# LSimon95/megatts2

Hardware: AMD Instinct MI355X
Metric: mel-frames/sec (whole node) (higher is better)
Workload: dtype f32; 1 GPU; C3: B=32/GPU x 1 GPU, Np=70, Tp=431, Tm=431; stages vqpe+mrte+adm+plm+decoder+vocoder; forced durations; weights=synthetic (name-seeded), parallelism=dp1 (utterance shards, one RCCL all-gather of mels per step)

## Files before the change

### include/megatts2_hip.h

```cpp
#ifndef MEGATTS2_HIP_H
#define MEGATTS2_HIP_H

#include <stddef.h>
#include <stdint.h>

#ifdef __cplusplus
extern "C" {
#endif

typedef struct mt2_model mt2_model;

typedef struct mt2_config {
    int32_t mel_bins, mrte_hidden, mrte_kernel, mrte_stride, mrte_n_layer, mrte_n_stack, mrte_n_block;
    int32_t content_ff_dim, content_n_heads, content_n_layers, phone_vocab;
    int32_t vq_mel_bins, vq_stride, vq_hidden, vq_kernel, vq_n_layers, vq_n_stacks, vq_n_blocks, vq_bins, vq_dim;
    int32_t dec_kernel, dec_hidden, dec_n_stack, dec_n_block;
    int32_t plm_layers, plm_heads, plm_vq_dim, plm_tc_dim, plm_bins;
    int32_t adm_layers, adm_heads, adm_emb_dim, adm_tc_dim, adm_tc_emb_dim;
    int32_t hg_in_dim, hg_init_channels, hg_n_up, hg_up_rates[8], hg_up_kernels[8];
    int32_t hg_n_res, hg_res_kernels[4], hg_res_dilations[4][3];
    float hg_slope;
    int32_t max_positions;
    int32_t hg_inference_padding;
    int32_t hg_reflect_pad;
// ... 230 lines not shown
enum { MT2_ATTN_NONE = 0, MT2_ATTN_GENERIC = 1, MT2_ATTN_REG = 2, MT2_ATTN_DS = 3, MT2_ATTN_LDS = 4, MT2_ATTN_X6 = 5, MT2_ATTN_X3H = 6 };
typedef struct mt2_attn_desc {
    int32_t struct_bytes;
    const float* Q; int32_t ldq;
    const float* K; int32_t ldk;
    const float* V; int32_t ldv;
    float* O; int32_t ldo;
    const int32_t* q_start; const int32_t* q_len; const int32_t* kv_start; const int32_t* kv_len; const int32_t* o_start;
    int32_t u_qstride, u_qlen, u_kvstride, u_kvlen, u_ostride;
    int32_t B, H, D, max_qlen, max_kvlen; float scale;
    int32_t lds_min_qlen, x6_min_qlen, lds_waves, ds_short, x3h, o_planes;
    int32_t* range_flag;
    int32_t* kernel_out;
} mt2_attn_desc;
int mt2_op_attention_desc(void* stream, const mt2_attn_desc* d);
int mt2_attention_route(const mt2_attn_desc* d, int32_t* err, int32_t* kernel, int32_t* tmpl, int32_t* launch, long long* lds);
int mt2_gemm_trace_begin(mt2_model* m);
int mt2_gemm_trace_end(mt2_model* m, int cap, const char** names, int64_t* launches, double* flops, double* ms);
int mt2_gemm_trace_shapes(mt2_model* m, char* buf, int cap, int top);
int mt2_gemm_config_count(void);
const char* mt2_gemm_config_name(int idx);
int mt2_gemm_route(int M, int N, int K, int taps, int dil, int groups, int pro_act, int operands, int misaligned, int force_cfg,
                   int x3h, int* err, int* cfg, int* variant, long long* lds, int* planes);
int mt2_op_gemm_x3h_ln(void* stream, const float* X, int ldx, int Rx, int a_mul, int shift0, const float* W, const void* W3,
                       const void* Wh, const float* wh_inv, const float* bias, const float* R, int ldr, float* C, int ldc, int M, int N,
                       int K, int epi_act, int force_cfg, float* stat_out, int32_t* stat_nt, int32_t* stat_w, const float* ln_stat,
                       int ln_nt, int ln_w, const float* ln_s, float ln_eps);
int mt2_bench_gemm(void* stream, int M, int N, int K, int taps, int dil, int flags, int force_cfg, int iters,
                   int w_copies, float* avg_ms, char* cfg_name, int cfg_name_cap, double* sustained_ghz);

#ifdef __cplusplus
}
#endif
#endif
```

### megatts2_amd/csrc/capi.inc

```

#include <climits>

namespace mt2 {
extern thread_local std::string g_last_error;
void finalize_model(mt2_model& m);
}

using namespace mt2;

#define MT2_API_BEGIN try {
#define MT2_API_END                                 \
    ::CallScope::verdict_of_open_call();            \
    return 0;                                       \
    }                                               \
    catch (const std::exception& e) {               \
        g_last_error = e.what();                    \
        return -1;                                  \
    }                                               \
    catch (...) {                                   \
        g_last_error = "unknown error";             \
        return -1;                                  \
    }

enum Need { NEED_G = 1, NEED_ADM = 2, NEED_PLM = 4, NEED_VOC = 8 };
// ... 248 lines not shown
    if (n == "ar_groups") return &m->ar_groups;
    if (n == "adm_groups") return &m->adm_groups;
    if (n == "plm_groups") return &m->plm_groups;
    if (n == "force_gemm_config") return &m->opts.force_cfg;
    if (n == "t_ks4") return &m->opts.t_ks4;
    if (n == "t_ks2") return &m->opts.t_ks2;
    if (n == "t32") return &m->opts.t32;
    if (n == "t32x32") return &m->opts.t32x32;
    if (n == "t_x6_256") return &m->opts.t_x6_256;
    if (n == "t_x6_128") return &m->opts.t_x6_128;
    if (n == "t_x3h_128") return &m->opts.t_x3h_128;
    if (n == "x3h") return &m->opts.x3h;
    if (n == "x6_ks") return &m->opts.x6_ks;
    if (n == "voc_streams") return &m->opts.voc_streams;
    if (n == "ldr_prio") return &m->opts.ldr_prio;
    if (n == "skinny_rows") return &m->opts.skinny_rows;
    if (n == "skinny_nw") return &m->opts.skinny_nw;
    if (n == "skinny_pairs") return &m->opts.skinny_pairs;
    if (n == "attn_lds_min") return &m->opts.attn_lds_min;
    if (n == "attn_x6_min") return &m->opts.attn_x6_min;
    if (n == "ln_pairs_adm") return &m->opts.ln_pairs_adm;
    if (n == "ln_pairs_maxm") return &m->opts.ln_pairs_maxm;
    if (n == "a_planes") return &m->opts.a_planes;
    return nullptr;
}
static bool* option_flag(mt2_model* m, const std::string& n) {
    if (n == "splitk") return &m->opts.splitk;
    if (n == "stage_markers") return &m->opts.markers;
    if (n == "win_conv") return &m->opts.win_conv;
    if (n == "x6_conv") return &m->opts.x6_conv;
    if (n == "x6_gemm") return &m->opts.x6_gemm;
    if (n == "skinny_tm") return &m->opts.skinny_tm;
    if (n == "ldr64") return &m->opts.ldr64;
    return nullptr;
}
int mt2_set_option(mt2_model* m, const char* name, int value) {
    MT2_API_BEGIN
    MT2_REQUIRE(m != nullptr && name != nullptr, "null argument");
    std::lock_guard<std::mutex> lk(m->call_mutex);
    const std::string n(name);
    if (n == "ar_groups") MT2_REQUIRE(value >= 1 && value <= 8, "ar_groups must be in 1..8");
    if (int* p = option_slot(m, n)) *p = value;
    else if (bool* q = option_flag(m, n)) *q = value != 0;
    else throw Error("unknown option " + n);
    MT2_API_END
}
// ... 790 lines not shown
    p.X = (const float*)ptr(0, 512); p.ldx = Cin; p.Rx = M + taps * dil; p.a_mul = 1; p.taps = taps; p.dil = dil; p.Cin = Cin;
    p.W = (const float*)ptr(1, 0); p.ldw = K; p.C = (float*)ptr(2, 1024); p.ldc = N; p.M = M; p.N = N; p.K = K; p.groups = groups;
    p.strideX = (long long)p.Rx * Cin; p.strideW = (long long)N * K; p.strideC = (long long)M * N; p.strideB = N; p.strideR = (long long)M * N;
    p.pro_act = pro_act; p.out_scale = 1.0f;
    if (operands & 1) p.W3 = ptr(3, 1);
    if (operands & 2) { p.Wh = ptr(4, 2); p.wh_inv = (const float*)ptr(5, 0); }
    if (operands & 4) { p.Wtm = (const float*)ptr(6, 4); p.tm_kb = K / 64; }
    if (operands & 8) p.stat_out = (float*)ptr(7, 8);
    if (operands & 16) { p.ln_stat = (const float*)ptr(8, 16); p.ln_g = p.ln_b = (const float*)ptr(9, 0); p.ln_w = 64; p.ln_nt = K / 64; }
    if (operands & 32) { p.R = (const float*)ptr(10, 32); p.ldr = N; }
    if (operands & 64) p.rowbase = (const int*)ptr(11, 64);
    p.a_planes = (operands & 128) ? 1 : 0;
    p.c_planes = (operands & 256) ? 1 : 0;
    EngineOpts o;
    o.force_cfg = force_cfg;
    o.x3h = x3h;
    const GemmRoute r = gemm_route(p, o);
    if (err) *err = (int)r.err;
    if (cfg) *cfg = r.cfg;
    if (variant) *variant = r.variant;
    if (lds) *lds = (long long)r.lds;
    if (planes) *planes = (gemm_takes_planes(p, o) ? 1 : 0) | (gemm_writes_planes(p, o) ? 2 : 0);
    return 0;
}

int mt2_op_gemm(void* stream, const float* X, int ldx, int Rx, const int32_t* rowbase, int a_mul, int shift0,
                int taps, int dil, int Cin, const float* W, int ldw, const float* bias, const float* R, int ldr,
                const int32_t* valid, float* C, int ldc, int M, int N, int pro_act, float pro_slope, int epi_act,
                float out_scale, int force_cfg) {
    MT2_API_BEGIN
    GemmP p{};
    p.X = X; p.ldx = ldx; p.Rx = Rx; p.rowbase = rowbase; p.a_mul = a_mul ? a_mul : 1; p.shift0 = shift0;
    p.taps = taps; p.dil = dil; p.Cin = Cin; p.W = W; p.ldw = ldw; p.bias = bias; p.R = R; p.ldr = ldr;
    p.valid = valid; p.C = C; p.ldc = ldc; p.M = M; p.N = N; p.K = taps * Cin; p.groups = 1;
    p.pro_act = pro_act; p.pro_slope = pro_slope; p.epi_act = epi_act; p.out_scale = out_scale;
    EngineOpts o;
    o.force_cfg = force_cfg;
    MT2_HIP(launch_gemm(p, (hipStream_t)stream, &o));
    MT2_API_END
}

int mt2_op_gemm_x6(void* stream, const float* X, int ldx, int Rx, int shift0, int taps, int dil, int Cin, const float* W,
                   const void* W3, const float* bias, const float* R, int ldr, const int32_t* valid, float* C, int ldc,
                   int M, int N, int pro_act, float pro_slope, int epi_act, int force_cfg) {
    MT2_API_BEGIN
    GemmP p{};
// ... 522 lines not shown
```

### megatts2_amd/csrc/gemm_x3h.hip

```cpp
#include "gemm_common.h"

#include <atomic>

#ifndef MT2_X3H_ABLATE
#define MT2_X3H_ABLATE 0
#endif
#define MT2_ABL_NOINGEST (MT2_X3H_ABLATE == 2 || MT2_X3H_ABLATE == 5 || MT2_X3H_ABLATE == 6 || MT2_X3H_ABLATE == 7)
#define MT2_ABL_NOSPLIT (MT2_X3H_ABLATE == 3 || MT2_X3H_ABLATE == 5 || MT2_X3H_ABLATE == 6)
#define MT2_ABL_NOBARRIER (MT2_X3H_ABLATE == 6 || MT2_X3H_ABLATE == 7)
#ifdef MT2_X3H_NO_BUFFER_LOADS
#define MT2_BUFFER_LOADS false
#else
#define MT2_BUFFER_LOADS true
#endif

namespace mt2 {

typedef _Float16 f16x8 __attribute__((ext_vector_type(8)));
typedef _Float16 f16x2 __attribute__((ext_vector_type(2)));
typedef float f32x2 __attribute__((ext_vector_type(2)));
typedef unsigned u32x4 __attribute__((ext_vector_type(4)));

constexpr float kX3hLoScale = 2048.0f, kX3hLoInv = 1.0f / 2048.0f, kX3hMaxIn = 65504.0f;

// ... 999 lines not shown
                    __builtin_amdgcn_s_barrier();
                    asm volatile("" ::: "memory");
                }
                fetch_a(b, sa, swza);
                fetch_b(b, sb);
                __builtin_amdgcn_sched_barrier(0);
            }
        }
        stn = stn + 1 == NST ? 0 : stn + 1;
        if (++qn == QS) { qn = 0; ++tapn; }
    };
    for (int c = 0; c + 1 < nk; ++c) chunk(std::false_type{});
    chunk(std::true_type{});
#pragma unroll
    for (int i = 0; i < TM; ++i)
#pragma unroll
        for (int j = 0; j < TN; ++j)
#pragma unroll
            for (int e = 0; e < 16; ++e) acc[i][j][e] = __builtin_fmaf(acl[i][j][e], kX3hLoInv, acc[i][j][e]) * inv_s[j];
    if (epilogue_t4_ok(p)) epilogue_t4<TM, TN>(p, acc, 0, m0 + wm * WTM, wn * WTN, lane);
    else epilogue<TM, TN>(p, acc, 0, m0 + wm * WTM, wn * WTN, lane);
}


#define MT2_X3H_LDR(IDX_, BM_, BN_, WM_, WN_, NL_, NST_)                                                                    \
    { IDX_, BM_, BN_, (WM_* WN_ + NL_) * 64, (size_t)NST_ * ((size_t)BM_ * BK * 4 + (size_t)(2 * BN_ / 16) * 1024),         \
      "x3hldr" #BM_ "x" #BN_ "_" #WM_ "x" #WN_ "+" #NL_ "_s" #NST_ "xc",                                                    \
      { gemm_x3h_ldr_kernel<BM_, BN_, WM_, WN_, NL_, NST_, ACT_NONE>, gemm_x3h_ldr_kernel<BM_, BN_, WM_, WN_, NL_, NST_, ACT_RELU>, \
        gemm_x3h_ldr_kernel<BM_, BN_, WM_, WN_, NL_, NST_, ACT_LRELU>, gemm_x3h_ldr_kernel<BM_, BN_, WM_, WN_, NL_, NST_, PRO_APL>, \
        gemm_x3h_ldr_kernel<BM_, BN_, WM_, WN_, NL_, NST_, PRO_LNX> }, PIPE_X3H, 0, 0, (BN_) / (WN_) }
#define MT2_X3H_KS(IDX_, BM_, BN_, WM_, WN_, KS_, NL_, NST_)                                                                \
    { IDX_, BM_, BN_, (WM_* WN_ * KS_ + NL_) * 64, (size_t)KS_ * NST_ * ((size_t)BM_ * BK * 4 + (size_t)(2 * BN_ / 16) * 1024), \
      "x3hks" #BM_ "x" #BN_ "_" #WM_ "x" #WN_ "_k" #KS_ "+" #NL_ "_s" #NST_,                                                \
      { gemm_x3h_ks_kernel<BM_, BN_, WM_, WN_, KS_, NL_, NST_, ACT_NONE>, gemm_x3h_ks_kernel<BM_, BN_, WM_, WN_, KS_, NL_, NST_, ACT_RELU>, \
        gemm_x3h_ks_kernel<BM_, BN_, WM_, WN_, KS_, NL_, NST_, ACT_LRELU>, gemm_x3h_ks_kernel<BM_, BN_, WM_, WN_, KS_, NL_, NST_, PRO_APL>, \
        gemm_x3h_ks_kernel<BM_, BN_, WM_, WN_, KS_, NL_, NST_, PRO_LNX> }, PIPE_X3H, 0, KS_, 32 }
#define MT2_X3H_WIN(IDX_, QS_, BM_, BN_, WM_, WN_, NST_, NL_)                                                               \
    { IDX_, BM_, BN_, (WM_* WN_ + NL_) * 64, (size_t)NST_ * (((2 * BN_ / 16 + NL_ - 1) / NL_) * NL_ * 1024),                  \
      "x3hwin" #BM_ "x" #BN_ "_" #WM_ "x" #WN_ "+" #NL_ "_s" #NST_,                                                          \
      { conv_win_x3h_kernel<QS_, BM_, BN_, WM_, WN_, NST_, ACT_NONE, NL_>, conv_win_x3h_kernel<QS_, BM_, BN_, WM_, WN_, NST_, ACT_RELU, NL_>, \
        conv_win_x3h_kernel<QS_, BM_, BN_, WM_, WN_, NST_, ACT_LRELU, NL_> }, PIPE_X3H, QS_ }

static const TileCfg kX3hRows[] = {
    MT2_X3H_KS(CFG_X3HKS32x64_K4, 32, 64, 1, 2, 4, 8, 2),
    MT2_X3H_KS(CFG_X3HKS64x64_K2, 64, 64, 2, 2, 2, 8, 3),
    MT2_X3H_KS(CFG_X3HKS32x32_K8, 32, 32, 1, 1, 8, 8, 2),
// ... 9 lines not shown
```

### megatts2_amd/csrc/model_stages.hip

```cpp
#include "mt2_model.h"
#include "x3h_planes.h"
#include "gemm_tiles.h"

#include <algorithm>
#include <cmath>
#include <cstring>
#include <numeric>

namespace mt2 {



static RowSet make_rows(const int* lens, int B, int G) {
    RowSet rs;
    rs.B = B; rs.G = G;
    rs.len.assign(lens, lens + B);
    rs.off.resize(B);
    int r = G;
    for (int b = 0; b < B; ++b) {
        MT2_REQUIRE(lens[b] >= 0, "negative utterance length");
        rs.off[b] = r;
        r += lens[b] + G;
        rs.maxlen = std::max(rs.maxlen, lens[b]);
    }
// ... 149 lines not shown
    }
    const bool planes = linear_takes_planes(c, h_scratch, K, M, w.W, w.bias, N, K, y, ldy, epi_act);
    LnP q{};
    q.x = x + (long long)shift0 * ldx; q.ldx = ldx * p.a_mul; q.gamma = w.g; q.beta = w.b; q.out = h_scratch; q.ldo = K;
    q.M = M; q.C = K; q.eps = 1e-5f; q.act = ACT_NONE; q.out_planes = planes ? 1 : 0; q.x3h_flag = c.m.opts.x3h_flag;
    MT2_HIP(launch_layernorm(q, c.s));
    linear(c, h_scratch, K, M, w.W, w.bias, N, K, y, ldy, nullptr, 0, nullptr, epi_act, planes, c_planes);
}
static LnOps ln1_qkv(const EncLayerW& w, int d, int n0 = 0) {
    return ln_ops(w.ln1g, w.ln1b, w.wqkv, w.bqkv, w.wqkv_l, w.sqkv, w.cqkv, n0, d);
}
static LnOps ln2_ff0(const EncLayerW& w, int d) {
    return ln_ops(w.ln2g, w.ln2b, w.ff0w, w.ff0b, w.ff0_l, w.sff0, w.cff0, 0, d);
}

static void conv_same(const Ctx& c, const float* x, int ldx, int R, const ConvW& w, float* y, int ldy,
                      const int* valid, int pro_act = ACT_NONE, float slope = 0.f, int epi_act = ACT_NONE,
                      const float* Rsd = nullptr, int ldr = 0, int dil = 1) {
    GemmP p{};
    p.X = x; p.ldx = ldx; p.Rx = R; p.taps = w.k; p.dil = dil; p.shift0 = -((w.k - 1) / 2) * dil; p.Cin = w.cin;
    p.W = w.w; p.bias = w.b; p.R = Rsd; p.ldr = ldr; p.valid = valid; p.C = y; p.ldc = ldy; p.M = R; p.N = w.cout;
    p.pro_act = pro_act; p.pro_slope = slope; p.epi_act = epi_act;
    gemm(c, p);
}

static void layernorm(const Ctx& c, const float* x, int ldx, const float* g, const float* b, int M, int C,
                      float* out, int ldo, const int* valid = nullptr, int valid_rows = 0,
                      const float* R1 = nullptr, int ldr1 = 0, int r1_rows = 0, int rows_per_group = 0,
                      int act = ACT_NONE, bool out_planes = false) {
    LnP p{};
    p.x = x; p.ldx = ldx; p.gamma = g; p.beta = b; p.rows_per_group = rows_per_group;
    p.R1 = R1; p.ldr1 = ldr1; p.r1_rows = r1_rows; p.valid = valid; p.valid_rows = valid_rows;
    p.out = out; p.ldo = ldo; p.M = M; p.C = C; p.eps = 1e-5f; p.act = act;
    p.out_planes = out_planes ? 1 : 0; p.x3h_flag = c.m.opts.x3h_flag;
    MT2_HIP(launch_layernorm(p, c.s));
}

static float* run_stack(const Ctx& c, const StackW& w, const float* x_in, bool shared_in, int R,
                        const int* valid) {
    const int C = w.C, G = w.groups;
    const size_t per = (size_t)R * C;
    float* T = c.ws.get<float>(per * G);
    float* Y = c.ws.get<float>(per * G);
    float* XA = c.ws.get<float>(per * G);
    float* XB = c.ws.get<float>(per * G);
    const float* cur = x_in;
// ... 991 lines not shown
        const int nside = m.opts.voc_streams > 1 ? 2 : 0;
        ensure_aux(m, nside);
        if (reflect) {
            int g0 = 0;
            for (int j = 0; j < 3; ++j) g0 = std::max(g0, (m.hg_res[i * 3 + j].k - 1) / 2 * m.hg_res[i * 3 + j].dil[0]);
            halo(c, up, ch, g0);
        }
        if (nside) {
            MT2_HIP(hipEventRecord(m.ev_fork, c.s));
            m.aux_forked = true;
            for (int j = 0; j < nside; ++j) MT2_HIP(hipStreamWaitEvent(m.aux_streams[j], m.ev_fork, 0));
        }
        for (int j = 0; j < 3; ++j) {
            const ResW& r = m.hg_res[i * 3 + j];
            const Ctx cj{m, (nside && j > 0) ? m.aux_streams[j - 1] : c.s, c.ws};
            float* t1 = c.ws.get<float>(per);
            float* ha = c.ws.get<float>(per);
            float* hb = c.ws.get<float>(per);
            rb[j] = c.ws.get<float>(per);
            const float* h = up;
            for (int n = 0; n < 3; ++n) {
                float* out = n == 2 ? rb[j] : (n == 0 ? ha : hb);
                if (n > 0) halo(cj, const_cast<float*>(h), ch, (r.k - 1) / 2 * r.dil[n]);
                conv_same(cj, h, ch, (int)R, r.c1[n], t1, ch, valid, ACT_LRELU, slope, ACT_LRELU, nullptr, 0, r.dil[n]);
                halo(cj, t1, ch, (r.k - 1) / 2);
                conv_same(cj, t1, ch, (int)R, r.c2[n], out, ch, valid, ACT_NONE, slope, ACT_NONE, h, ch, 1);
                h = out;
            }
        }
        for (int j = 0; j < nside; ++j) {
            MT2_HIP(hipEventRecord(m.ev_join[j], m.aux_streams[j]));
            MT2_HIP(hipStreamWaitEvent(c.s, m.ev_join[j], 0));
        }
        if (!reflect && i + 1 == cfg.hg_n_up && m.hg_post.cout == 1 && (ch & 3) == 0 && ch <= 128 && m.hg_post.k <= 15) {
            float* wav = c.ws.get<float>((size_t)R);
            const hipError_t e = launch_conv_post(rb[0], rb[1], rb[2], 1.0f / 3.0f, R, ch, m.hg_post.k, m.hg_post.w,
                                                  m.hg_post.b, 0.01f, valid, wav, c.s);
            if (e == hipSuccess) return wav;
            if (e != hipErrorNotSupported) MT2_HIP(e);
        }
        x = c.ws.get<float>(per);
        MT2_HIP(launch_avg3(rb[0], rb[1], rb[2], 1.0f / 3.0f, x, (long long)per, c.s));
    }
    float* wav = c.ws.get<float>((size_t)R);
    halo(c, x, ch, (m.hg_post.k - 1) / 2);
    conv_same(c, x, ch, (int)R, m.hg_post, wav, 1, valid, ACT_LRELU, 0.01f, ACT_TANH);
// ... 617 lines not shown
```

### megatts2_amd/csrc/mt2_kernels.h

```cpp
#pragma once
#include <hip/hip_runtime.h>
#include <stdint.h>

#include <atomic>
#include <vector>

namespace mt2 {

inline hipError_t dyn_lds_once(std::atomic<unsigned long long>& done, const void* fn, size_t bytes) {
    int dev = 0;
    hipError_t e = hipGetDevice(&dev);
    if (e != hipSuccess) return e;
    const unsigned long long bit = 1ull << (dev & 63);
    if (done.load(std::memory_order_acquire) & bit) return hipSuccess;
    e = hipFuncSetAttribute(fn, hipFuncAttributeMaxDynamicSharedMemorySize, (int)bytes);
    if (e != hipSuccess) return e;
    done.fetch_or(bit, std::memory_order_release);
    return hipSuccess;
}

constexpr int kInvalidRow = -(1 << 30);

enum Act : int { ACT_NONE = 0, ACT_RELU = 1, ACT_LRELU = 2, ACT_TANH = 3,
                 ACT_LOGCLAMP = 4 };
// ... 20 lines not shown
    const float* Wtm = nullptr;
    int tm_n0 = 0, tm_k0 = 0;
    int tm_kb = 0;
    const float* bias; long long strideB;
    const float* R; long long strideR; int ldr;
    const int* valid;
    float* C; long long strideC; int ldc;
    int M, N, K, groups;
    int pro_act; float pro_slope; int epi_act; float out_scale;
    const float* ln_g; const float* ln_b; float ln_eps;
    float* stat_out = nullptr; int stat_nt = 0, stat_w = 0;
    const float* ln_stat = nullptr; int ln_nt = 0, ln_w = 0;
};
struct TraceRec { int cfg; double flops; hipEvent_t e0, e1; int M, N, K, groups; };
struct EngineOpts {
    int force_cfg = -1;
    int t_ks4 = 256, t_ks2 = 640, t32 = 64, t32x32 = 160;
    bool splitk = true;
    int voc_streams = 3;
    bool win_conv = true;
    bool x6_conv = true;
    bool x6_gemm = true;
    int x3h = 15;
    int* x3h_flag = nullptr;
    int t_x3h_128 = 72;
    int t_x6_256 = 160, t_x6_128 = 72;
    int x6_ks = 4;
    int a_planes = 3;
    bool ldr64 = false;
    int ldr_prio = 3;
    int skinny_rows = 64;
    int attn_lds_min = 640;
    int attn_x6_min = 192;
    bool skinny_tm = true;
    int skinny_pairs = 1;
    int skinny_nw = 16;
    bool markers = false;
    bool trace_on = false;
    std::vector<TraceRec> trace;
    const char* last_cfg = "";
    int last_stat_nt = 0, last_stat_w = 0;
    int ln_pairs = 0;
    int ln_pairs_adm = 2;
    int ln_pairs_maxk = 1024;
    int ln_pairs_maxm = 1280;
};
struct GemmRoute { hipError_t err; int cfg; int variant; size_t lds; int stat_nt, stat_w; };
GemmRoute gemm_route(const GemmP& p, const EngineOpts& o);
hipError_t launch_gemm(const GemmP& p, hipStream_t s, EngineOpts* o = nullptr);
bool gemm_takes_planes(const GemmP& p, const EngineOpts& o);
bool gemm_writes_planes(const GemmP& p, const EngineOpts& o);
bool gemm_skinny_eligible(const GemmP& p, int max_rows);
hipError_t launch_gemm_skinny(const GemmP& p, hipStream_t s);
bool gemm_skinny_tm_eligible(const GemmP& p, int max_rows);
hipError_t launch_gemm_skinny_tm(const GemmP& p, hipStream_t s);
hipError_t launch_tile_major(const float* W, int N, int K, float* out, hipStream_t s);
int gemm_num_configs();
const char* gemm_config_name(int idx);
int gemm_trace_collect(EngineOpts& o, int cap, const char** names, int64_t* launches, double* flops, double* ms);
int gemm_trace_shapes(EngineOpts& o, char* buf, int cap, int top);

struct LnP {
    const float* x; int ldx;
    const float* gamma; const float* beta; int rows_per_group;
    const float* R1; int ldr1; int r1_rows; const float* R2; int ldr2;
    const int* valid; int valid_rows;
    float* out; int ldo;
    int M, C; float eps; int act;
    int out_planes = 0;
    int* x3h_flag = nullptr;
};
hipError_t launch_layernorm(const LnP& p, hipStream_t s);
// ... 196 lines not shown
```

### megatts2_amd/runtime.py

```python
from __future__ import annotations

import ctypes as C
import math
import os
from typing import Dict, Optional, Sequence

import numpy as np

from . import config as cfgmod
from . import sampling as sampmod

_LIB = None
MAX_POSITIONS = 8192

MT2_RUN_PLM, MT2_RUN_VOCODER, MT2_SKIP_ADM, MT2_PROMPT_VQPE = 1, 2, 4, 8
ACT_NONE, ACT_RELU, ACT_LRELU, ACT_TANH = 0, 1, 2, 3
ACT_LOGCLAMP = 4
MT2_RESAMPLE_NORMALIZE = 1
TRIM_FRAME, TRIM_HOP = 2048, 512
F0_FRAME, F0_WINDOW, F0_MAX_LAG = 1024, 768, 256
DTW_MAX_LEN, DTW_DIR_COLS = 4096, 16


class NativeError(RuntimeError):
# ... 908 lines not shown
    inv = torch.empty(w.shape[0], dtype=torch.float32)
    _check(lib.mt2_x3h_split(C.c_void_p(w.data_ptr()), C.c_longlong(w.shape[0]), C.c_longlong(w.shape[1]),
                             C.c_void_p(planes.data_ptr()), C.c_void_p(inv.data_ptr())))
    return planes, inv


def op_conv_x3h(X, W, bias=None, R=None, valid=None, shift0=0, taps=1, dil=1, Cin=None, pro_act=ACT_NONE, pro_slope=0.0,
                epi_act=ACT_NONE, force_cfg=-1, want_flag=False):
    import torch
    lib = load_library()
    Cin = Cin or X.shape[1]
    N, M = W.shape[0], X.shape[0]
    W3 = split_bf16x3(W).to(X.device)
    ph, inv = split_f16x2_rows(W)
    ph, inv = ph.to(X.device), inv.to(X.device)
    out = torch.empty(M, N, device=X.device, dtype=torch.float32)
    flag = torch.zeros(4, device=X.device, dtype=torch.int32)
    _check(lib.mt2_op_gemm_x3h(_stream(), _ptr(X), X.shape[1], M, shift0, taps, dil, Cin, _ptr(W), _ptr(W3), _ptr(ph), _ptr(inv),
                               _ptr(bias), _ptr(R), R.shape[1] if R is not None else 0, _ptr(valid), _ptr(out), N, M, N, pro_act,
                               C.c_float(pro_slope), epi_act, force_cfg, _ptr(flag)))
    return (out, int(flag[0].item())) if want_flag else out


def op_gemm_x6_ln(X, W, bias=None, R=None, M=None, a_mul=1, shift0=0, epi_act=ACT_NONE, force_cfg=-1, want_stats=False,
                  ln=None, eps=1e-5, x3h=False):
    import torch
    lib = load_library()
    K, N = X.shape[1], W.shape[0]
    M = M or X.shape[0]
    dev = X.device
    out = torch.empty(M, N, device=dev, dtype=torch.float32)
    stat = torch.zeros(M, 32, 2, device=dev, dtype=torch.float32) if want_stats else None
    nt, pw = C.c_int32(0), C.c_int32(0)
    ln_stat, ln_nt, ln_w, ln_s = None, 0, 0, None
    if ln is not None:
        gamma, beta, pairs, ln_w = ln
        Wd = W.double().cpu()
        Wl = (W.cpu() * gamma.cpu()[None, :]).to(torch.float32)
        ln_s = Wl.double().sum(1).to(torch.float32).to(dev)
        bias = (Wd @ beta.double().cpu() + (bias.double().cpu() if bias is not None else 0.0)).to(torch.float32).to(dev)
        W = Wl.to(dev)
        ln_stat = pairs.contiguous()
        ln_nt = pairs.shape[1]
    W = W.contiguous()
    W3 = split_bf16x3(W).to(dev)
    if x3h:
# ... 348 lines not shown
```

Measured before the change: 78320 mel-frames/s.

## Fuse HiFiGAN resblock conv pairs into one x3h kernel keeping intermediate in LDS

Adds a conv_pair kernel that runs a resblock's two consecutive convolutions (leaky-relu conv with dilation, then conv plus residual) in one launch. The intermediate activation stays in LDS as f16 hi/lo planes, and dedicated loader waves stream both weight sets. This removes one launch, the global write and read of the intermediate, and the halo pass. The cost is recomputing overlapping rows at tile edges (output tile BM-(taps-1)). The path is on by default for 32- and 64-channel resblocks (pair_fuse=3) and falls back to the old path when a case is unsupported.

```diff
diff --git a/include/megatts2_hip.h b/include/megatts2_hip.h
--- a/include/megatts2_hip.h
+++ b/include/megatts2_hip.h
@@ -276,6 +276,11 @@
 const char* mt2_gemm_config_name(int idx);
 int mt2_gemm_route(int M, int N, int K, int taps, int dil, int groups, int pro_act, int operands, int misaligned, int force_cfg,
                    int x3h, int* err, int* cfg, int* variant, long long* lds, int* planes);
+int mt2_conv_pair_route(int R, int C, int taps, int dil, int flags, int pair_fuse, int x3h, int* err, long long* lds, int* grid,
+                        int* block, int* bm, int* bmo);
+int mt2_op_conv_pair(void* stream, const float* X, int ldx, int R, int C, int taps, int dil, float slope, const void* Wh1,
+                     const float* inv1, const float* bias1, const void* Wh2, const float* inv2, const float* bias2,
+                     const int32_t* valid, float* Y, int ldy, int pair_fuse, int32_t* range_flag);
 int mt2_op_gemm_x3h_ln(void* stream, const float* X, int ldx, int Rx, int a_mul, int shift0, const float* W, const void* W3,
                        const void* Wh, const float* wh_inv, const float* bias, const float* R, int ldr, float* C, int ldc, int M, int N,
                        int K, int epi_act, int force_cfg, float* stat_out, int32_t* stat_nt, int32_t* stat_w, const float* ln_stat,
diff --git a/megatts2_amd/csrc/capi.inc b/megatts2_amd/csrc/capi.inc
--- a/megatts2_amd/csrc/capi.inc
+++ b/megatts2_amd/csrc/capi.inc
@@ -294,6 +294,7 @@
     if (n == "ln_pairs_adm") return &m->opts.ln_pairs_adm;
     if (n == "ln_pairs_maxm") return &m->opts.ln_pairs_maxm;
     if (n == "a_planes") return &m->opts.a_planes;
+    if (n == "pair_fuse") return &m->opts.pair_fuse;
     return nullptr;
 }
 static bool* option_flag(mt2_model* m, const std::string& n) {
@@ -1130,6 +1131,45 @@
     if (lds) *lds = (long long)r.lds;
     if (planes) *planes = (gemm_takes_planes(p, o) ? 1 : 0) | (gemm_writes_planes(p, o) ? 2 : 0);
     return 0;
+}
+
+int mt2_conv_pair_route(int R, int C, int taps, int dil, int flags, int pair_fuse, int x3h, int* err, long long* lds, int* grid,
+                        int* block, int* bm, int* bmo) {
+    alignas(128) static char dummy[8 * 128];
+    PairP p{};
+    p.X = (const float*)dummy; p.ldx = C; p.R = R; p.C = C; p.taps = taps; p.dil = dil; p.slope = 0.1f;
+    if (!(flags & 2)) { p.Wh1 = dummy + 128; p.inv1 = (const float*)(dummy + 256); p.Wh2 = dummy + 384; p.inv2 = (const float*)(dummy + 512); }
+    p.bias1 = (const float*)(dummy + 640); p.bias2 = (const float*)(dummy + 768);
+    p.wh_ldb = 4ll * (((long long)taps * C + 31) / 32 * 32);
+    p.Y = (float*)(dummy + 896 + ((flags & 8) ? 4 : 0)); p.ldy = C;
+    p.reflect = (flags & 1) ? 1 : 0;
+    if ((flags & 4) && R > 0) p.ldx = (int)((((1ll << 31) / 4 + R - 1) / R + 3) & ~3ll);
+    EngineOpts o;
+    o.pair_fuse = pair_fuse;
+    o.x3h = x3h;
+    const PairRoute r = conv_pair_route(p, o);
+    if (err) *err = (int)r.err;
+    if (lds) *lds = (long long)r.lds;
+    if (grid) *grid = (int)r.grid;
+    if (block) *block = (int)r.block;
+    if (bm) *bm = r.bm;
+    if (bmo) *bmo = r.bmo;
+    return 0;
+}
+int mt2_op_conv_pair(void* stream, const float* X, int ldx, int R, int C, int taps, int dil, float slope, const void* Wh1,
+                     const float* inv1, const float* bias1, const void* Wh2, const float* inv2, const float* bias2,
+                     const int32_t* valid, float* Y, int ldy, int pair_fuse, int32_t* range_flag) {
+    MT2_API_BEGIN
+    PairP p{};
+    p.X = X; p.ldx = ldx; p.R = R; p.C = C; p.taps = taps; p.dil = dil; p.slope = slope;
+    p.Wh1 = Wh1; p.inv1 = inv1; p.bias1 = bias1; p.Wh2 = Wh2; p.inv2 = inv2; p.bias2 = bias2;
+    p.wh_ldb = 4ll * (((long long)taps * C + 31) / 32 * 32);
+    p.valid = valid; p.Y = Y; p.ldy = ldy;
+    EngineOpts o;
+    o.pair_fuse = pair_fuse;
+    o.x3h_flag = range_flag;
+    MT2_HIP(launch_conv_pair(p, (hipStream_t)stream, &o));
+    MT2_API_END
 }
 
 int mt2_op_gemm(void* stream, const float* X, int ldx, int Rx, const int32_t* rowbase, int a_mul, int shift0,
diff --git a/megatts2_amd/csrc/gemm_x3h.hip b/megatts2_amd/csrc/gemm_x3h.hip
--- a/megatts2_amd/csrc/gemm_x3h.hip
+++ b/megatts2_amd/csrc/gemm_x3h.hip
@@ -1045,6 +1045,375 @@
     else epilogue<TM, TN>(p, acc, 0, m0 + wm * WTM, wn * WTN, lane);
 }
 
+template <int PRO, int QS, int NT, int MAXT>
+__device__ __forceinline__ void pair_rows_to_planes(float* win, int tid, int WRp, int nrows, float slope, float& amax) {
+    const unsigned lds_w = (unsigned)(unsigned long long)(__attribute__((address_space(3))) float*)win;
+    const int ntask = QS * nrows * 4;
+    f32x4 in[MAXT][2];
+    int rbk_[MAXT];
+    __builtin_amdgcn_s_barrier();
+    asm volatile("" ::: "memory");
+#pragma unroll
+    for (int u = 0; u < MAXT; ++u) {
+        const int t = tid + u * NT;
+        const int tt = t < ntask ? t : 0;
+        const int rr = tt >> 2, j = tt & 3;
+        const int q = rr / nrows, row = rr - q * nrows;
+        const int rbk = q * WRp + row;
+        rbk_[u] = rbk;
+        const int swz = (row >> 1) & 7;
+        const unsigned base = lds_w + (unsigned)rbk * 128;
+        in[u][0] = lds_read_b128(base + (unsigned)(((2 * j) ^ swz) * 16));
+        in[u][1] = lds_read_b128(base + (unsigned)(((2 * j + 1) ^ swz) * 16));
+    }
+    asm volatile("s_waitcnt lgkmcnt(0)" ::: "memory");
+#pragma unroll
+    for (int u = 0; u < MAXT; ++u) asm volatile("" : "+v"(in[u][0]), "+v"(in[u][1]));
+    __builtin_amdgcn_s_barrier();
+    asm volatile("" ::: "memory");
+#pragma unroll
+    for (int u = 0; u < MAXT; ++u) {
+        const int t = tid + u * NT;
+        if (t < ntask) {
+            const int j = t & 3, rbk = rbk_[u];
+            const int swz = ((rbk % WRp) >> 1) & 7;
+            u32x4 ph, pl;
+            split2_f16<PRO>(in[u][0], in[u][1], slope, ph, pl, amax);
+            char* dst = reinterpret_cast<char*>(win) + (size_t)rbk * 128;
+            *reinterpret_cast<u32x4*>(dst + ((j ^ swz) * 16)) = ph;
+            *reinterpret_cast<u32x4*>(dst + (((4 + j) ^ swz) * 16)) = pl;
+        }
+    }
+    asm volatile("s_waitcnt lgkmcnt(0)" ::: "memory");
+}
+
+template <int QS, int BM, int BN, int WGM, int WGN, int NST, int NL>
+__global__ __launch_bounds__((WGM * WGN + NL) * 64) void conv_pair_x3h_kernel(PairP p) {
+    constexpr int NW = WGM * WGN;
+    constexpr int WTM = BM / WGM, WTN = BN / WGN;
+    constexpr int TM = WTM / 32, TN = WTN / 32;
+    constexpr int BPIECES = BN / 8;
+    constexpr int NI = NL;
+    constexpr int B_IT = (BPIECES + NI - 1) / NI;
+    constexpr int STAGE_B = B_IT * NI * 1024;
+    constexpr int NT = (NW + NL) * 64;
+    constexpr int MAXT1 = (QS * (BM + 64) * 4 + NT - 1) / NT;
+    constexpr int MAXT2 = (QS * BM * 4 + NT - 1) / NT;
+    static_assert(NL > 0 && WTM % 32 == 0 && WTN % 32 == 0 && NST >= 3 && (NST - 2) * B_IT < 64 && BN == 32 * QS, "config");
+
+    extern __shared__ __attribute__((aligned(16))) float smem[];
+    const int tid = threadIdx.x, lane = tid & 63;
+    const int wave_all = __builtin_amdgcn_readfirstlane(tid >> 6);
+    const bool loader = wave_all >= NW;
+    const int wave = loader ? wave_all - NW : wave_all;
+    const int wm = wave / WGN, wn = wave % WGN;
+    const int taps = p.taps;
+    const int WR = BM + (taps - 1) * p.dil, WRp = (WR + 7) & ~7;
+    const int BMo = BM - (taps - 1);
+    char* ring = reinterpret_cast<char*>(smem);
+    float* win = smem + NST * STAGE_B / 4;
+
+    const int ntm = (p.R + BMo - 1) / BMo;
+    const int bid = blockIdx.x;
+    const int xcd = bid & 7, qq = ntm >> 3, rr = ntm & 7;
+    const int tile = (xcd < rr ? xcd * (qq + 1) : rr * (qq + 1) + (xcd - rr) * qq) + (bid >> 3);
+    const int o0 = tile * BMo;
+    const int t0 = o0 - (taps - 1) / 2;
+
+    const float* __restrict__ X = p.X;
+    const long long zoff_x = (const float*)g_zero16 - X;
+    const int ldx = p.ldx, Rx = p.R;
+    {
+        const int lrow = lane >> 3;
+        const int ppq = WRp >> 3, pieces = QS * ppq;
+        const int row_first = t0 - (taps - 1) / 2 * p.dil;
+        for (int pc = wave_all; pc < pieces; pc += NW + NL) {
+            const int q = pc / ppq, r8 = pc - q * ppq;
+            const int row = r8 * 8 + lrow;
+            const int grow = row_first + row;
+            const int slot = (lane & 7) ^ ((row >> 1) & 7);
+            const bool ok = (row < WR) & ((unsigned)grow < (unsigned)Rx);
+            const long long off = ok ? (long long)grow * ldx + q * 32 + slot * 4 : zoff_x;
+            __builtin_amdgcn_global_load_lds((const __attribute__((address_space(1))) void*)(X + off),
+                                             (__attribute__((address_space(3))) void*)(win + (q * WRp + r8 * 8) * 32), 16, 0, 0);
+        }
+    }
+    const int nk = taps * QS;
+    constexpr unsigned kOut = 0x80000000u;
+    unsigned vob[B_IT];
+#pragma unroll
+    for (int j = 0; j < B_IT; ++j) {
+        const int pc = j * NI + wave;
+        const int n = pc * 8 + (lane >> 3);
+        const int sl = (lane & 7) ^ ((n >> 1) & 7);
+        vob[j] = (pc < BPIECES && n < BN) ? (unsigned)(n * (int)p.wh_ldb + sl * 16) : kOut;
+    }
+    auto issue = [&](const __amdgpu_buffer_rsrc_t& rs, int c, int st) __attribute__((always_inline)) {
+        char* Bs = ring + st * STAGE_B + wave * 1024;
+#pragma unroll
+        for (int j = 0; j < B_IT; ++j)
+            __builtin_amdgcn_raw_ptr_buffer_load_lds(rs, (__attribute__((address_space(3))) void*)(Bs + j * NI * 1024), 16, (int)vob[j], c * 128, 0, 0);
+    };
+    auto loader_loop = [&](const __amdgpu_buffer_rsrc_t& rs) __attribute__((always_inline)) {
+        for (int c = 0; c < nk; ++c) {
+            if (c == 0) { if (NST - 2 < nk) wait_vmcnt<(NST - 2) * B_IT>(); else wait_vmcnt<0>(); }
+            else if (c + NST - 3 < nk) wait_vmcnt<(NST - 3) * B_IT>();
+            else wait_vmcnt<0>();
+            __builtin_amdgcn_s_barrier();
+            if (c >= 1 && c + NST - 2 < nk) issue(rs, c + NST - 2, (c + NST - 2) % NST);
+        }
+    };
+    if (loader) {
+        const __amdgpu_buffer_rsrc_t rs1 = __builtin_amdgcn_make_buffer_rsrc(const_cast<char*>(reinterpret_cast<const char*>(p.Wh1)), 0, (int)kOut, 0x00020000);
+        const __amdgpu_buffer_rsrc_t rs2 = __builtin_amdgcn_make_buffer_rsrc(const_cast<char*>(reinterpret_cast<const char*>(p.Wh2)), 0, (int)kOut, 0x00020000);
+        loader_priority(p.ldr_prio);
+#pragma unroll
+        for (int st = 0; st < NST - 1; ++st)
+            if (st < nk) issue(rs1, st, st);
+        if (nk >= NST - 1) wait_vmcnt<(NST - 1) * B_IT>();
+        else wait_vmcnt<0>();
+        float amax = 0.0f;
+        pair_rows_to_planes<ACT_LRELU, QS, NT, MAXT1>(win, tid, WRp, WRp, p.slope, amax);
+        if (p.x3h_flag != nullptr && __builtin_amdgcn_ballot_w64(amax >= kX3hMaxIn) != 0ull && lane == 0) atomicOr(p.x3h_flag, 1);
+        loader_loop(rs1);
+        __builtin_amdgcn_s_barrier();
+        asm volatile("" ::: "memory");
+#pragma unroll
+        for (int st = 0; st < NST - 1; ++st)
+            if (st < nk) issue(rs2, st, st);
+        amax = 0.0f;
+        pair_rows_to_planes<ACT_NONE, QS, NT, MAXT2>(win, tid, WRp, BM, p.slope, amax);
+        if (p.x3h_flag != nullptr && __builtin_amdgcn_ballot_w64(amax >= kX3hMaxIn) != 0ull && lane == 0) atomicOr(p.x3h_flag, 1);
+        loader_loop(rs2);
+        return;
+    }
+    unsigned vmask[TM];
+    {
+        int vv[TM];
+#pragma unroll
+        for (int i = 0; i < TM; ++i) {
+            const int g = t0 + wm * WTM + i * 32 + (lane & 31);
+            const bool ok = (unsigned)g < (unsigned)Rx;
+            vv[i] = ok ? (p.valid ? p.valid[g] : 1) : 0;
+        }
+        wait_vmcnt<0>();
+#pragma unroll
+        for (int i = 0; i < TM; ++i) vmask[i] = (unsigned)__builtin_amdgcn_ballot_w64(vv[i] != 0);
+    }
+    float amax = 0.0f;
+    pair_rows_to_planes<ACT_LRELU, QS, NT, MAXT1>(win, tid, WRp, WRp, p.slope, amax);
+    if (p.x3h_flag != nullptr && __builtin_amdgcn_ballot_w64(amax >= kX3hMaxIn) != 0ull && lane == 0) atomicOr(p.x3h_flag, 1);
+
+    f32x16 acc[TM][TN], acl[TM][TN];
+    const int half = lane >> 5;
+    const unsigned lds_ring = (unsigned)(unsigned long long)(__attribute__((address_space(3))) char*)ring;
+    const unsigned lds_win = (unsigned)(unsigned long long)(__attribute__((address_space(3))) float*)win;
+    const int nrow = wn * WTN + (lane & 31);
+    const unsigned b_lane = lds_ring + nrow * 128;
+    const int swzb = (nrow >> 1) & 7;
+    unsigned koffb[2][2];
+#pragma unroll
+    for (int b = 0; b < 2; ++b) {
+        koffb[b][0] = (unsigned)(((b * 2 + half) ^ swzb) * 16);
+        koffb[b][1] = (unsigned)(((4 + b * 2 + half) ^ swzb) * 16);
+    }
+    const int arow0 = wm * WTM + (lane & 31);
+    constexpr int N1 = 2 * TM + 2 * TN;
+    static_assert(N1 <= 15, "lgkmcnt is four bits wide");
+    u32x4 ra[2][TM][2];
+    u32x4 rb[2][2][TN];
+    auto fetch_a = [&](int b, unsigned sa, int swza) __attribute__((always_inline)) {
+        const unsigned vh = sa + (unsigned)(((b * 2 + half) ^ swza) * 16), vl = sa + (unsigned)(((4 + b * 2 + half) ^ swza) * 16);
+        static_for(std::make_integer_sequence<int, TM>{}, [&](auto ic) {
+            constexpr int i = decltype(ic)::value;
+            ra[b][i][0] = __builtin_bit_cast(u32x4, lds_read_b128_imm<i * 32 * BK * 4>(vh));
+            ra[b][i][1] = __builtin_bit_cast(u32x4, lds_read_b128_imm<i * 32 * BK * 4>(vl));
+        });
+    };
+    auto fetch_b = [&](int b, unsigned sb) __attribute__((always_inline)) {
+        const unsigned vb0 = sb + koffb[b][0], vb1 = sb + koffb[b][1];
+        static_for(std::make_integer_sequence<int, TN>{}, [&](auto ic) {
+            constexpr int j = decltype(ic)::value;
+            rb[b][0][j] = __builtin_bit_cast(u32x4, lds_read_b128_imm<j * 32 * 128>(vb0));
+            rb[b][1][j] = __builtin_bit_cast(u32x4, lds_read_b128_imm<j * 32 * 128>(vb1));
+        });
+    };
+    auto tie_set = [&](int b) __attribute__((always_inline)) {
+#pragma unroll
+        for (int i = 0; i < TM; ++i) asm volatile("" : "+v"(ra[b][i][0]), "+v"(ra[b][i][1]));
+#pragma unroll
+        for (int pl = 0; pl < 2; ++pl)
+#pragma unroll
+            for (int j = 0; j < TN; ++j) asm volatile("" : "+v"(rb[b][pl][j]));
+    };
+    auto products = [&](int b) __attribute__((always_inline)) {
+#pragma unroll
+        for (int i = 0; i < TM; ++i) {
+            const f16x8 Ah = __builtin_bit_cast(f16x8, ra[b][i][0]), Al = __builtin_bit_cast(f16x8, ra[b][i][1]);
+#pragma unroll
+            for (int j = 0; j < TN; ++j)
+                acl[i][j] = __builtin_amdgcn_mfma_f32_32x32x16_f16(Ah, __builtin_bit_cast(f16x8, rb[b][1][j]), acl[i][j], 0, 0, 0);
+#pragma unroll
+            for (int j = 0; j < TN; ++j)
+                acc[i][j] = __builtin_amdgcn_mfma_f32_32x32x16_f16(Ah, __builtin_bit_cast(f16x8, rb[b][0][j]), acc[i][j], 0, 0, 0);
+#pragma unroll
+            for (int j = 0; j < TN; ++j)
+                acl[i][j] = __builtin_amdgcn_mfma_f32_32x32x16_f16(Al, __builtin_bit_cast(f16x8, rb[b][0][j]), acl[i][j], 0, 0, 0);
+        }
+    };
+    auto kloop = [&](const int dil, const float* __restrict__ wh_inv) __attribute__((always_inline)) {
+        float inv_s[TN];
+#pragma unroll
+        for (int j = 0; j < TN; ++j) inv_s[j] = wh_inv[wn * WTN + j * 32 + (lane & 31)];
+#pragma unroll
+        for (int i = 0; i < TM; ++i)
+#pragma unroll
+            for (int j = 0; j < TN; ++j)
+#pragma unroll
+                for (int e = 0; e < 16; ++e) { acc[i][j][e] = 0.0f; acl[i][j][e] = 0.0f; }
+        __builtin_amdgcn_s_barrier();
+        asm volatile("" ::: "memory");
+        {
+            const unsigned sa0 = lds_win + (unsigned)(arow0 * BK) * 4;
+            const int swz0 = (arow0 >> 1) & 7;
+            fetch_a(0, sa0, swz0); fetch_b(0, b_lane); fetch_a(1, sa0, swz0); fetch_b(1, b_lane);
+        }
+        __builtin_amdgcn_sched_barrier(0);
+        int stn = 1 % NST, tapn = 0, qn = 1;
+        if (qn == QS) { qn = 0; tapn = 1; }
+        auto chunk = [&](auto last_c) __attribute__((always_inline)) {
+            constexpr bool last = decltype(last_c)::value;
+            const int arow = arow0 + tapn * dil;
+            const int swza = (arow >> 1) & 7;
+            const unsigned sa = lds_win + (unsigned)((qn * WRp + arow) * BK) * 4;
+            const unsigned sb = b_lane + (unsigned)stn * STAGE_B;
+#pragma unroll
+            for (int b = 0; b < 2; ++b) {
+                if (last && b == 1) asm volatile("s_waitcnt lgkmcnt(0)" ::: "memory");
+                else asm volatile("s_waitcnt lgkmcnt(%0)" :: "n"(N1) : "memory");
+                tie_set(b);
+                __builtin_amdgcn_sched_barrier(0);
+                products(b);
+                __builtin_amdgcn_sched_barrier(0);
+                if constexpr (!last) {
+                    if (b == 0) {
+                        __builtin_amdgcn_s_barrier();
+                        asm volatile("" ::: "memory");
+                    }
+                    fetch_a(b, sa, swza);
+                    fetch_b(b, sb);
+                    __builtin_amdgcn_sched_barrier(0);
+                }
+            }
+            stn = stn + 1 == NST ? 0 : stn + 1;
+            if (++qn == QS) { qn = 0; ++tapn; }
+        };
+        for (int c = 0; c + 1 < nk; ++c) chunk(std::false_type{});
+        chunk(std::true_type{});
+#pragma unroll
+        for (int i = 0; i < TM; ++i)
+#pragma unroll
+            for (int j = 0; j < TN; ++j)
+#pragma unroll
+                for (int e = 0; e < 16; ++e) {
+                    float v = __builtin_fmaf(acl[i][j][e], kX3hLoInv, acc[i][j][e]) * inv_s[j];
+                    asm volatile("" : "+v"(v));
+                    acc[i][j][e] = v;
+                }
+    };
+    kloop(p.dil, p.inv1);
+    {
+        float b1[TN];
+#pragma unroll
+        for (int j = 0; j < TN; ++j) b1[j] = p.bias1 ? p.bias1[wn * WTN + j * 32 + (lane & 31)] : 0.0f;
+        const float slope = p.slope;
+        __builtin_amdgcn_s_barrier();
+        asm volatile("" ::: "memory");
+        const int c = lane & 31;
+#pragma unroll
+        for (int i = 0; i < TM; ++i)
+#pragma unroll
+            for (int e = 0; e < 16; ++e) {
+                const int r32 = (e & 3) + 8 * (e >> 2) + 4 * half;
+                const int row = wm * WTM + i * 32 + r32;
+                const bool on = (vmask[i] >> r32) & 1u;
+                float* dst = win + row * 32 + ((((c >> 2) ^ ((row >> 1) & 7)) << 2) | (c & 3));
+#pragma unroll
+                for (int j = 0; j < TN; ++j) {
+                    float v = acc[i][j][e] + b1[j];
+                    v = v >= 0.0f ? v : v * slope;
+                    dst[((wn * WTN) / 32 + j) * WRp * 32] = on ? v : 0.0f;
+                }
+            }
+        asm volatile("s_waitcnt lgkmcnt(0)" ::: "memory");
+    }
+    amax = 0.0f;
+    pair_rows_to_planes<ACT_NONE, QS, NT, MAXT2>(win, tid, WRp, BM, p.slope, amax);
+    if (p.x3h_flag != nullptr && __builtin_amdgcn_ballot_w64(amax >= kX3hMaxIn) != 0ull && lane == 0) atomicOr(p.x3h_flag, 1);
+    kloop(1, p.inv2);
+    GemmP e{};
+    e.bias = p.bias2; e.R = p.X; e.ldr = p.ldx; e.valid = p.valid; e.C = p.Y; e.ldc = p.ldy;
+    e.M = min(p.R, o0 + BMo); e.N = BN; e.epi_act = ACT_NONE; e.pro_slope = p.slope; e.out_scale = 1.0f;
+    if (epilogue_t4_ok(e)) epilogue_t4<TM, TN>(e, acc, 0, o0 + wm * WTM, wn * WTN, lane);
+    else epilogue<TM, TN>(e, acc, 0, o0 + wm * WTM, wn * WTN, lane);
+}
+
+typedef void (*PairKernel)(PairP);
+struct PairTile { int C, bm, threads; size_t ring; PairKernel fn; };
+#define MT2_PAIR_TILE(QS_, BM_, BN_, WM_, WN_, NST_, NL_)                                                                    \
+    { BN_, BM_, (WM_* WN_ + NL_) * 64, (size_t)NST_ * (((2 * BN_ / 16 + NL_ - 1) / NL_) * NL_ * 1024),                        \
+      conv_pair_x3h_kernel<QS_, BM_, BN_, WM_, WN_, NST_, NL_> }
+static const PairTile kPairTiles[3] = {
+    MT2_PAIR_TILE(1, 256, 32, 8, 1, 4, 4), MT2_PAIR_TILE(2, 256, 64, 8, 1, 4, 4), MT2_PAIR_TILE(4, 128, 128, 4, 2, 3, 4),
+};
+
+PairRoute conv_pair_route(const PairP& p, const EngineOpts& o) {
+    PairRoute r{hipSuccess, -1, 0, 0, 0, 0, 0};
+    const auto fail = [&r](hipError_t e) { r.err = e; r.tile = -1; r.lds = 0; r.grid = r.block = 0; r.bm = r.bmo = 0; return r; };
+    if (p.R <= 0) return r;
+    if (p.taps < 2 || p.dil < 1 || p.C <= 0) return fail(hipErrorInvalidValue);
+    const int t = p.C == 32 ? 0 : (p.C == 64 ? 1 : (p.C == 128 ? 2 : -1));
+    if (t < 0 || !((o.pair_fuse >> t) & 1)) return fail(hipErrorNotSupported);
+    if (p.reflect || (long long)(p.taps - 1) * p.dil > 64) return fail(hipErrorNotSupported);
+    if (!o.win_conv || !o.x6_conv || !(o.x3h & 4) || o.force_cfg >= 0 || o.ldr64) return fail(hipErrorNotSupported);
+    if (!p.Wh1 || !p.Wh2 || !p.inv1 || !p.inv2) return fail(hipErrorNotSupported);
+    const long long two_g = 1ll << 31;
+    if ((long long)p.R * p.ldx * 4 >= two_g || (long long)p.R * p.ldy * 4 >= two_g || (long long)p.C * p.wh_ldb >= two_g - 1)
+        return fail(hipErrorNotSupported);
+    if (!p.X || !p.Y || p.ldx < p.C || p.ldy < p.C || p.wh_ldb < 4ll * p.taps * p.C) return fail(hipErrorInvalidValue);
+    if (((p.ldx | p.ldy) & 3) || (p.wh_ldb & 127) || (((unsigned long long)p.Wh1 | (unsigned long long)p.Wh2) & 127) ||
+        (((unsigned long long)p.X | (unsigned long long)p.Y | (unsigned long long)p.bias1 | (unsigned long long)p.bias2) & 15))
+        return fail(hipErrorNotSupported);
+    const PairTile& c = kPairTiles[t];
+    const int wrp = (c.bm + (p.taps - 1) * p.dil + 7) & ~7;
+    r.tile = t;
+    r.bm = c.bm;
+    r.bmo = c.bm - (p.taps - 1);
+    r.lds = c.ring + (size_t)(p.C / 32) * wrp * BK * sizeof(float);
+    r.grid = (unsigned)((p.R + r.bmo - 1) / r.bmo);
+    r.block = (unsigned)c.threads;
+    return r;
+}
+
+static std::atomic<unsigned long long> g_pair_attr_done[3];
+
+hipError_t launch_conv_pair(const PairP& p_in, hipStream_t s, EngineOpts* opts) {
+    static const EngineOpts kDefaults;
+    const EngineOpts& o = opts ? *opts : kDefaults;
+    const PairRoute r = conv_pair_route(p_in, o);
+    if (r.err != hipSuccess || r.grid == 0) return r.err;
+    const PairTile& c = kPairTiles[r.tile];
+    PairP p = p_in;
+    p.x3h_flag = o.x3h_flag;
+    p.ldr_prio = o.ldr_prio;
+    const size_t lds_attr = c.ring + (size_t)(p.C / 32) * ((c.bm + 64 + 7) & ~7) * BK * sizeof(float);
+    const hipError_t e = dyn_lds_once(g_pair_attr_done[r.tile], reinterpret_cast<const void*>(c.fn), lds_attr);
+    if (e != hipSuccess) return e;
+    if (opts) opts->last_cfg = "x3hpair";
+    hipLaunchKernelGGL(c.fn, dim3(r.grid), dim3(r.block), r.lds, s, p);
+    return hipGetLastError();
+}
+
 
 #define MT2_X3H_LDR(IDX_, BM_, BN_, WM_, WN_, NL_, NST_)                                                                    \
     { IDX_, BM_, BN_, (WM_* WN_ + NL_) * 64, (size_t)NST_ * ((size_t)BM_ * BK * 4 + (size_t)(2 * BN_ / 16) * 1024),         \
diff --git a/megatts2_amd/csrc/model_stages.hip b/megatts2_amd/csrc/model_stages.hip
--- a/megatts2_amd/csrc/model_stages.hip
+++ b/megatts2_amd/csrc/model_stages.hip
@@ -195,6 +195,27 @@
     p.W = w.w; p.bias = w.b; p.R = Rsd; p.ldr = ldr; p.valid = valid; p.C = y; p.ldc = ldy; p.M = R; p.N = w.cout;
     p.pro_act = pro_act; p.pro_slope = slope; p.epi_act = epi_act;
     gemm(c, p);
+}
+
+static bool conv_pair(const Ctx& c, const float* x, int C, int R, const ConvW& w1, const ConvW& w2, int dil, float slope,
+                      bool reflect, float* y, const int* valid) {
+    if (w1.k != w2.k || w1.cin != C || w1.cout != C || w2.cin != C || w2.cout != C) return false;
+    GemmP g1{}, g2{};
+    g1.W = w1.w; g1.taps = w1.k; g1.Cin = C; g1.groups = 1;
+    g2.W = w2.w; g2.taps = w2.k; g2.Cin = C; g2.groups = 1;
+    attach_planes(c.m, g1);
+    attach_planes(c.m, g2);
+    if (!g1.W3 || !g2.W3 || g1.wh_ldb != g2.wh_ldb) return false;
+    PairP p{};
+    p.X = x; p.ldx = C; p.R = R; p.C = C; p.taps = w1.k; p.dil = dil; p.slope = slope;
+    p.Wh1 = g1.Wh; p.inv1 = g1.wh_inv; p.bias1 = w1.b;
+    p.Wh2 = g2.Wh; p.inv2 = g2.wh_inv; p.bias2 = w2.b;
+    p.wh_ldb = g1.wh_ldb ? g1.wh_ldb : 4ll * ((w1.k * C + 31) / 32 * 32);
+    p.valid = valid; p.Y = y; p.ldy = C; p.reflect = reflect ? 1 : 0;
+    const hipError_t e = launch_conv_pair(p, c.s, &c.m.opts);
+    if (e == hipErrorNotSupported) return false;
+    MT2_HIP(e);
+    return true;
 }
 
 static void layernorm(const Ctx& c, const float* x, int ldx, const float* g, const float* b, int M, int C,
@@ -1232,6 +1253,10 @@
             for (int n = 0; n < 3; ++n) {
                 float* out = n == 2 ? rb[j] : (n == 0 ? ha : hb);
                 if (n > 0) halo(cj, const_cast<float*>(h), ch, (r.k - 1) / 2 * r.dil[n]);
+                if (m.opts.pair_fuse && conv_pair(cj, h, ch, (int)R, r.c1[n], r.c2[n], r.dil[n], slope, reflect, out, valid)) {
+                    h = out;
+                    continue;
+                }
                 conv_same(cj, h, ch, (int)R, r.c1[n], t1, ch, valid, ACT_LRELU, slope, ACT_LRELU, nullptr, 0, r.dil[n]);
                 halo(cj, t1, ch, (r.k - 1) / 2);
                 conv_same(cj, t1, ch, (int)R, r.c2[n], out, ch, valid, ACT_NONE, slope, ACT_NONE, h, ch, 1);
diff --git a/megatts2_amd/csrc/mt2_kernels.h b/megatts2_amd/csrc/mt2_kernels.h
--- a/megatts2_amd/csrc/mt2_kernels.h
+++ b/megatts2_amd/csrc/mt2_kernels.h
@@ -66,6 +66,7 @@
     bool x6_conv = true;
     bool x6_gemm = true;
     int x3h = 15;
+    int pair_fuse = 3;
     int* x3h_flag = nullptr;
     int t_x3h_128 = 72;
     int t_x6_256 = 160, t_x6_128 = 72;
@@ -92,6 +93,22 @@
 struct GemmRoute { hipError_t err; int cfg; int variant; size_t lds; int stat_nt, stat_w; };
 GemmRoute gemm_route(const GemmP& p, const EngineOpts& o);
 hipError_t launch_gemm(const GemmP& p, hipStream_t s, EngineOpts* o = nullptr);
+struct PairP {
+    const float* X; int ldx;
+    int R, C, taps, dil;
+    float slope;
+    const void* Wh1; const float* inv1; const float* bias1;
+    const void* Wh2; const float* inv2; const float* bias2;
+    long long wh_ldb;
+    const int* valid;
+    float* Y; int ldy;
+    int reflect = 0;
+    int* x3h_flag = nullptr;
+    int ldr_prio = 0;
+};
+struct PairRoute { hipError_t err; int tile; size_t lds; unsigned grid, block; int bm, bmo; };
+PairRoute conv_pair_route(const PairP& p, const EngineOpts& o);
+hipError_t launch_conv_pair(const PairP& p, hipStream_t s, EngineOpts* o = nullptr);
 bool gemm_takes_planes(const GemmP& p, const EngineOpts& o);
 bool gemm_writes_planes(const GemmP& p, const EngineOpts& o);
 bool gemm_skinny_eligible(const GemmP& p, int max_rows);
diff --git a/megatts2_amd/runtime.py b/megatts2_amd/runtime.py
--- a/megatts2_amd/runtime.py
+++ b/megatts2_amd/runtime.py
@@ -954,6 +954,28 @@
     return (out, int(flag[0].item())) if want_flag else out
 
 
+def op_conv_pair(X, W1, b1, W2, b2, taps, dil, slope, valid=None, channels=None, out=None, pair_fuse=7, want_flag=False):
+    import torch
+    lib = load_library()
+    Cc = channels or X.shape[1]
+    R = X.shape[0]
+    p1, i1 = (t.to(X.device) for t in split_f16x2_rows(W1))
+    p2, i2 = (t.to(X.device) for t in split_f16x2_rows(W2))
+    if out is None:
+        out = torch.empty(R, Cc, device=X.device, dtype=torch.float32)
+    flag = torch.zeros(4, device=X.device, dtype=torch.int32)
+    _check(lib.mt2_op_conv_pair(_stream(), _ptr(X), X.shape[1], R, Cc, taps, dil, C.c_float(slope), _ptr(p1), _ptr(i1), _ptr(b1),
+                                _ptr(p2), _ptr(i2), _ptr(b2), _ptr(valid), _ptr(out), out.shape[1], pair_fuse, _ptr(flag)))
+    return (out, int(flag[0].item())) if want_flag else out
+
+
+def op_conv_pair_route(R, Cn, taps, dil, flags=0, pair_fuse=7, x3h=15):
+    err, lds, grid, block, bm, bmo = C.c_int(0), C.c_longlong(0), C.c_int(0), C.c_int(0), C.c_int(0), C.c_int(0)
+    load_library().mt2_conv_pair_route(R, Cn, taps, dil, flags, pair_fuse, x3h, C.byref(err), C.byref(lds), C.byref(grid), C.byref(block),
+                                       C.byref(bm), C.byref(bmo))
+    return {"err": err.value, "lds": lds.value, "grid": grid.value, "block": block.value, "bm": bm.value, "bmo": bmo.value}
+
+
 def op_gemm_x6_ln(X, W, bias=None, R=None, M=None, a_mul=1, shift0=0, epi_act=ACT_NONE, force_cfg=-1, want_stats=False,
                   ln=None, eps=1e-5, x3h=False):
     import torch
```

Result: faster. 79360 mel-frames/s (median of 6 runs) (+1.3%).
